# andrewhou1/GeomConsistentFR

Hardware: AMD Instinct MI355X
Metric: ray_steps_per_sec (higher is better)
Workload: dtype f64+f32

## Files before the change

### geomconsistentfr_amd/csrc/gcfr_march.hpp

```cpp
#pragma once

#include "gcfr_device.hpp"
#include "gcfr_mutants.hpp"

#include "../../include/gcfr.h"

#include <atomic>
#include <cstddef>
#include <type_traits>

namespace gcfr {

struct ShadowArgs {
    const float *depth;
    const uint8_t *mask;
    const float *light_pt;
    const double *t_table;
    float *min_dist;
    int32_t *argmin;
    int32_t mask_batch, L, H, W, N;
    int32_t tiles_x, tiles_per_image;
    float bonus, bx_lo, bx_hi, by_lo, by_hi;
};

struct RayConst {
    float x, y, zb;
    float dx, dy;
    float BCx, BCy, BCz;
    double x64, y64, dx64, dy64, halfW, halfH;
    int H, W;
};

__device__ inline float ray_sample(const RayConst &rc, double t, __amdgpu_buffer_rsrc_t zr,
                                   __amdgpu_buffer_rsrc_t mr, bool &masked)
{
    const int W = rc.W, H = rc.H;
    const double sx = rc.x64 + t * rc.dx64;
    const double sy = rc.y64 + t * rc.dy64;
    const int col_r = (int)(__builtin_rint(sx) + rc.halfW);
    const int row_r = (int)(rc.halfH - __builtin_rint(sy));
    const double ux = (sx + rc.halfW) - 0.0001;
    const double uy = (rc.halfH - sy) - 0.0001;
    const double fxd = __builtin_floor(ux), gxd = __builtin_ceil(ux);
    const double fyd = __builtin_floor(uy), gyd = __builtin_ceil(uy);
    int fx = (int)fxd, gx = (int)gxd, fy = (int)fyd, gy = (int)gyd;
    const double wx0 = gxd - ux, wx1 = ux - fxd;
    const double wy0 = gyd - uy, wy1 = uy - fyd;
    fx += (fx >> 31) & W;
    fy += (fy >> 31) & H;
    const int rowf = fy * W, rowg = gy * W;
    const double zUL = buf_load_f32(zr, (rowf + fx) << 2);
    const double zUR = buf_load_f32(zr, (rowf + gx) << 2);
    const double zLL = buf_load_f32(zr, (rowg + fx) << 2);
    const double zLR = buf_load_f32(zr, (rowg + gx) << 2);
    const uint32_t mk = buf_load_u8(mr, row_r * W + col_r);
    const double up = zUL * wx0 + zUR * wx1;
    const double low = zLL * wx0 + zLR * wx1;
    const double zA = up * wy0 + low * wy1;
    const float Ax = (float)(ux - rc.halfW), Ay = (float)(rc.halfH - uy), Az = (float)zA;
    const float BAx = Ax - rc.x, BAy = Ay - rc.y, BAz = Az - rc.zb;
    const float Xx = __builtin_fmaf(BAy, rc.BCz, -(BAz * rc.BCy));
    const float Xy = __builtin_fmaf(BAz, rc.BCx, -(BAx * rc.BCz));
    const float Xz = __builtin_fmaf(BAx, rc.BCy, -(BAy * rc.BCx));
    masked = (mk == 0);
    return ((Xx * Xx + Xy * Xy) + Xz * Xz) + kEps4;
}

__device__ inline int first_tied_sample(const RayConst &rc, const double *t_table, __amdgpu_buffer_rsrc_t zr,
                                        __amdgpu_buffer_rsrc_t mr, bool tie, int prevk, float den, float d)
{
    int first = prevk;
    int k_hi = tie ? prevk : 0;
    for (int off = 32; off > 0; off >>= 1)
        k_hi = max(k_hi, __shfl_xor(k_hi, off));
    k_hi = __builtin_amdgcn_readfirstlane(k_hi);
    bool found = !tie;
    for (int k = 0; k < k_hi; ++k) {
        bool masked;
        const float S = ray_sample(rc, t_table[k], zr, mr, masked);
        const bool hit = !found && (k < prevk) && !masked && (__builtin_sqrtf(S) / den == d);
        first = hit ? k : first;
        found = found || hit;
    }
    return first;
}



struct PrepassLights {
    const float *light_raw = nullptr;
    float *unit_out = nullptr, *light_pt_out = nullptr;
    int L = 0, clamp_z = 0;
    float clamp_min = 0.0f, light_distance = 0.0f;
};

constexpr int kBBoxInit = 0x7f7f7f7f;

template <int CTRL, int ROW_MASK>
__device__ inline int dpp_min_step(int v)
{
    const int moved = __builtin_amdgcn_update_dpp(0x7fffffff, v, CTRL, ROW_MASK, 0xf, false);
    return min(v, moved);
}
__device__ inline int wave_min_i32(int v)
{
    v = dpp_min_step<0x111, 0xf>(v);
    v = dpp_min_step<0x112, 0xf>(v);
    v = dpp_min_step<0x114, 0xf>(v);
    v = dpp_min_step<0x118, 0xf>(v);
    v = dpp_min_step<0x142, 0xa>(v);
    v = dpp_min_step<0x143, 0xc>(v);
    return __builtin_amdgcn_readlane(v, 63);
}

__device__ inline int f32_sortable(float f)
{
    const int i = __builtin_bit_cast(int, f);
    return i ^ ((i >> 31) & 0x7fffffff);
}
__device__ inline float f32_unsortable(int i)
{
    return __builtin_bit_cast(float, i ^ ((i >> 31) & 0x7fffffff));
}

template <class TablePtrT>
__device__ inline int zb_log2_stride(int H, int W, int N, TablePtrT t_table, int group, bool *fits = nullptr)
{
    if (fits)
        *fits = false;
    if (N < 2)
        return 3;
    const float step = fabsf((float)((t_table[N - 1] - t_table[0]) / (double)(N - 1)));
    const float fd = (float)(group - 1) * step * (float)max(H, W) * 1.002f;
    const int need = (int)fminf(fmaxf(fd, 0.0f), 1024.0f) + GCFR_M(22, 1, 3);
    int ls = 3;
    while ((1 << ls) < need && ls < 5)
        ++ls;
    if (fits)
        *fits = (1 << ls) >= need;
    return ls;
}

__host__ __device__ inline int zb_max_tiles(int H, int W) { return ((H >> 3) + 1) * ((W >> 3) + 1) + 1; }
__host__ __device__ inline int zb_stride(int H, int W) { return (zb_max_tiles(H, W) + 63) & ~63; }
constexpr int kHorizonDim = 1024;
constexpr int kHorizonBands = 4;
__host__ __device__ inline bool hz_shape_ok(int H, int W) { return ((W & 3) == 0) && W <= kHorizonDim && H <= kHorizonDim; }
__host__ __device__ inline int zb_slot(int H, int W) { return hz_shape_ok(H, W) ? zb_stride(H, W) + 4 * kHorizonDim : zb_stride(H, W); }

__device__ inline float row_sum_f32(float v)
{
    v += __builtin_bit_cast(float, __builtin_amdgcn_update_dpp(0, __builtin_bit_cast(int, v), 0x111, 0xf, 0xf, false));
    v += __builtin_bit_cast(float, __builtin_amdgcn_update_dpp(0, __builtin_bit_cast(int, v), 0x112, 0xf, 0xf, false));
    v += __builtin_bit_cast(float, __builtin_amdgcn_update_dpp(0, __builtin_bit_cast(int, v), 0x114, 0xf, 0xf, false));
    v += __builtin_bit_cast(float, __builtin_amdgcn_update_dpp(0, __builtin_bit_cast(int, v), 0x118, 0xf, 0xf, false));
    return v;
}
__device__ inline float lane_value(float v, int lane)
{
    return __builtin_bit_cast(float, __builtin_amdgcn_readlane(__builtin_bit_cast(int, v), lane));
}


constexpr int kQueueSlot = 64;
enum { kTfOk = 0, kTfStride = 1, kTfTabs = 2, kTfTfirst = 3, kTfInvDt = 4 };
constexpr int kStatChunk = 16384;
__host__ __device__ inline int stat_chunk_shift(int H, int W)
{
    const int raw = (H * W + kStatChunk - 1) >> 14;
    return (raw > 8 && raw <= 16) ? 15 : 14;
}
__host__ __device__ inline int stat_chunk_px(int H, int W) { return 1 << stat_chunk_shift(H, W); }
__host__ __device__ inline int n_stat_chunks(int H, int W)
{
    const int sh = stat_chunk_shift(H, W);
    return (H * W + (1 << sh) - 1) >> sh;
}
static_assert(kStatChunk == 1 << 14, "stat_chunk_shift() spells kStatChunk as a shift");


struct MarchEpilogueArgs {
    float *min_dist;
    int32_t *argmin;
    float bonus, bx_lo, bx_hi, by_lo, by_hi;
    const float *normals;
    const float *albedo;
    const float *ambient;
    float *shadow_w, *full, *final_shading, *rendered;
    float intensity;
    NormalsArgs nrm;
    float *normals_out;
};

struct ShadowQuadArgs {
    const float *depth;
    const float4 *quad;
    const int *bbox;
    const int *diag;
    const float4 *zb;
    const int *zrange;
    const int *mones;
    int *tflag;
    const uint8_t *mask;
    const uint32_t *reserved0;
    const float *light_pt;
    const double *t_table;
    unsigned long long *counters;
    int32_t mask_batch, B, L, H, W, N;
    int32_t tiles_x, tiles_y;
    int32_t bl_offset;
    int32_t hz_off;
    MarchEpilogueArgs epi;
};

typedef const __attribute__((address_space(4))) ShadowQuadArgs *ArgPtr;
typedef const __attribute__((address_space(4))) MarchEpilogueArgs *EpiPtr;
__device__ __forceinline__ ArgPtr kernel_args()
{
    return (ArgPtr)__builtin_amdgcn_kernarg_segment_ptr();
}
template <class T>
__device__ __forceinline__ T launder(T p)
{
    asm volatile("" : "+s"(p));
    return p;
}

constexpr double kRintMagic = 6755399441055744.0;
typedef float f32x4 __attribute__((ext_vector_type(4)));

__device__ inline int lo32(double v)
{
    return (int)(unsigned)(__builtin_bit_cast(unsigned long long, v) & 0xffffffffull);
}

enum { kCntTiles, kCntGroupsNominal, kCntGroupsVisited, kCntBoundTests, kCntBodies, kCntLaneSamples, kCntEarlyExit,
       kCntTieRemarch, kCntSamplesInRange, kCntBoundsGivenUp, kCntVisitsAfterLastBody, kCntVisitsBeforeFirstBody,
       kCntTrailEnter, kCntTrailSkips, kCntTrailLeave, kCntRoughSamples, kCntWaveSamples, kCntWaveSamplesTaken, kCntLaneTakes,
       kCntAuditBoundChecks, kCntAuditBoundViol, kCntAuditTermChecks, kCntAuditTermViol, kCntAuditMaskedChecks, kCntAuditMaskedViol,
       kCntAuditSafeViol, kCntAuditMaxUse, kCntUsed };
static_assert(kCntUsed <= GCFR_N_COUNTERS, "gcfr_options.counters holds GCFR_N_COUNTERS tallies");
#if defined(GCFR_AUDIT) && !defined(GCFR_COUNTERS)
#error "-DGCFR_AUDIT needs -DGCFR_COUNTERS"
#endif
#ifdef GCFR_COUNTERS
#define GCFR_COUNT(i, n) (cnt[i] += (unsigned)(n))
#else
#define GCFR_COUNT(i, n) ((void)0)
#endif

struct ImageStats {
    int r_min, c_min, r_max, c_max;
    int s_min, s_max, d_min, d_max;
    int gz_lo_s, gz_nhi_s;
    int mask_all_ones;
};
__device__ inline ImageStats reduce_image_stats(ArgPtr a, int b, int lane, bool want_z)
{
    const int n = n_stat_chunks(a->H, a->W);
    if (n <= 8) {
        typedef const __attribute__((address_space(4))) int *ConstI32Ptr;
        const ConstI32Ptr sb = (ConstI32Ptr)(unsigned long long)a->bbox + 4 * (size_t)(a->mask_batch == 1 ? 0 : b) * n;
        const ConstI32Ptr sz = (ConstI32Ptr)(unsigned long long)a->zrange + 2 * (size_t)b * n;
        const ConstI32Ptr so = (ConstI32Ptr)(unsigned long long)a->mones + (size_t)(a->mask_batch == 1 ? 0 : b) * n;
        const ConstI32Ptr sd = (ConstI32Ptr)(unsigned long long)a->diag + 4 * (size_t)(a->mask_batch == 1 ? 0 : b) * n;
        int d0 = kBBoxInit, d1 = kBBoxInit, d2 = kBBoxInit, d3 = kBBoxInit;
        int m0 = kBBoxInit, m1 = kBBoxInit, m2 = kBBoxInit, m3 = kBBoxInit, z0 = 0x7fffffff, z1 = 0x7fffffff, ones = 1;
#pragma unroll
        for (int j = 0; j < 8; ++j) {
            if (j < n) {
                m0 = min(m0, sb[4 * j + 0]);
                m1 = min(m1, sb[4 * j + 1]);
                m2 = min(m2, sb[4 * j + 2]);
                m3 = min(m3, sb[4 * j + 3]);
                ones = min(ones, so[j]);
                d0 = min(d0, sd[4 * j + 0]);
                d1 = min(d1, sd[4 * j + 1]);
                d2 = min(d2, sd[4 * j + 2]);
                d3 = min(d3, sd[4 * j + 3]);
                if (want_z) {
                    z0 = min(z0, sz[2 * j + 0]);
                    z1 = min(z1, sz[2 * j + 1]);
                }
            }
        }
        ImageStats st;
        st.r_min = m0;
        st.c_min = m1;
        st.r_max = -m2;
        st.c_max = -m3;
        st.gz_lo_s = z0;
        st.gz_nhi_s = z1;
        st.mask_all_ones = ones;
        st.s_min = d0;
        st.s_max = -d1;
        st.d_min = d2;
        st.d_max = -d3;
        return st;
    }
    const int4 *pb = (const int4 *)a->bbox + (size_t)(a->mask_batch == 1 ? 0 : b) * n;
    const int2 *pz = (const int2 *)a->zrange + (size_t)b * n;
    const int *po = a->mones + (size_t)(a->mask_batch == 1 ? 0 : b) * n;
    const int4 *pd = (const int4 *)a->diag + (size_t)(a->mask_batch == 1 ? 0 : b) * n;
    int4 m = make_int4(kBBoxInit, kBBoxInit, kBBoxInit, kBBoxInit), dg = m;
    int2 mz = make_int2(0x7fffffff, 0x7fffffff);
    int ones = 1;
    for (int j = lane; j < n; j += 64) {
        ones = min(ones, po[j]);
        const int4 v = pb[j];
        m.x = min(m.x, v.x);
        m.y = min(m.y, v.y);
        m.z = min(m.z, v.z);
        m.w = min(m.w, v.w);
        const int4 w = pd[j];
        dg.x = min(dg.x, w.x);
        dg.y = min(dg.y, w.y);
        dg.z = min(dg.z, w.z);
        dg.w = min(dg.w, w.w);
        if (want_z) {
            const int2 vz = pz[j];
            mz.x = min(mz.x, vz.x);
            mz.y = min(mz.y, vz.y);
        }
    }
    ImageStats st;
    st.r_min = wave_min_i32(m.x);
    st.c_min = wave_min_i32(m.y);
    st.r_max = -wave_min_i32(m.z);
    st.c_max = -wave_min_i32(m.w);
    st.gz_lo_s = want_z ? wave_min_i32(mz.x) : 0x7fffffff;
    st.gz_nhi_s = want_z ? wave_min_i32(mz.y) : 0x7fffffff;
    st.mask_all_ones = wave_min_i32(ones);
    st.s_min = wave_min_i32(dg.x);
    st.s_max = -wave_min_i32(dg.y);
    st.d_min = wave_min_i32(dg.z);
    st.d_max = -wave_min_i32(dg.w);
    return st;
}

__device__ inline int fresh_lane_id()
{
    int l;
    asm volatile("v_mbcnt_lo_u32_b32 %0, -1, 0\n\tv_mbcnt_hi_u32_b32 %0, -1, %0" : "=v"(l));
    return l;
}

enum { kModeInline = 0, kModeFull = 1, kModeRough = 2 };
#ifndef GCFR_ROUGH_CHUNK
#define GCFR_ROUGH_CHUNK 3
#endif
#ifndef GCFR_ROUGH_CHUNK_ARGMIN
#define GCFR_ROUGH_CHUNK_ARGMIN 3
#endif
template <int TILE_W, bool EVEN_HALF, bool WANT_ARGMIN, int DEPTH, bool FUSE_SHADE, int SPLIT, bool ALL_ONES = false, bool OWN = false,
          int MODE = kModeInline>
__device__ __forceinline__ bool march_tile(ArgPtr a, const int bl, const int qy, const int tx,
                                           const ImageStats &st)
{
    static_assert(MODE == kModeInline || SPLIT == 0, "full / rough pairs: the grid schedule's kernels");
    constexpr int TILE_H = 64 / TILE_W;
    static_assert(SPLIT == 0 || SPLIT == 1, "SPLIT: 0 = one wave per tile, 1 = the workgroup's four waves split the sample range");
    static_assert(!(OWN && (SPLIT != 0 || ALL_ONES)), "pixels = mask: the grid schedule only");
    const int H = a->H, W = a->W, L = a->L;
    typedef const __attribute__((address_space(4))) double *TablePtr;
    typedef const __attribute__((address_space(4))) float *ConstF32Ptr;
    typedef const __attribute__((address_space(4))) int *ConstI32Ptr;
    const TablePtr tt = (TablePtr)(unsigned long long)a->t_table;
    const int lane = fresh_lane_id();
    const int wave = __builtin_amdgcn_readfirstlane((int)(threadIdx.x >> 6));
    constexpr bool KSPLIT = SPLIT == 1;
    constexpr bool TRAIL = !KSPLIT;
    constexpr bool ROUGH = MODE == kModeRough;
    const int chunk = KSPLIT ? (a->N + 3) >> 2 : a->N;
    const int k_lo = KSPLIT ? wave * chunk : 0;
    const int N = KSPLIT ? min(a->N, k_lo + chunk) : a->N;
#ifdef GCFR_COUNTERS
    unsigned cnt[kCntUsed] = {};
    unsigned cnt_since_body = 0, cnt_had_body = 0;
    const unsigned long long trace_t0 = __builtin_amdgcn_s_memrealtime(), trace_c0 = __builtin_amdgcn_s_memtime();
#endif

    const int b = bl / L;
    const int l = bl - b * L;
    int r = qy * TILE_H + lane / TILE_W;
    int c = tx * TILE_W + (lane % TILE_W);
    const bool valid = (r < H) && (c < W);
    r = valid ? r : H - 1;
    c = valid ? c : W - 1;

    const size_t P = (size_t)H * W;
    const int Wp = W + 1;
    const size_t Pq = (size_t)(H + 1) * Wp;
    const __amdgpu_buffer_rsrc_t qr = make_rsrc(a->quad + (size_t)b * Pq, (int)(Pq * 16));
    const __amdgpu_buffer_rsrc_t mr =
        make_rsrc(a->mask + (size_t)(a->mask_batch == 1 ? 0 : b) * P, (int)P);

    const bool own_off = GCFR_M(17, false &&, ) OWN && (!valid || (buf_load_u8(mr, __mul24(r, W) + c) == 0));

    const ConstF32Ptr lp = (ConstF32Ptr)(unsigned long long)a->light_pt;
    const float Cx = lp[3 * bl + 0], Cy = lp[3 * bl + 1], Cz = lp[3 * bl + 2];
    const Box box = image_box(H, W);
    const LightCase lc = classify_light(Cx, Cy, box);
    const float halfWf = W / 2.0f, halfHf = H / 2.0f;
    const double halfW = W / 2.0, halfH = H / 2.0;
    const int halfWi = W / 2, halfHi = H / 2;

    const float x = (float)c - halfWf, y = halfHf - (float)r;
    const float zb = a->depth[(size_t)b * P + (size_t)r * W + c];
    float Ex, Ey;
    end_point(x, y, Cx, Cy, box, lc, Ex, Ey);
    const float dxf = Ex - x, dyf = Ey - y;
    const float BCx = Cx - x, BCy = Cy - y, BCz = Cz - zb;
    const bool finite_ray = (dxf - dxf == 0.0f) && (dyf - dyf == 0.0f);
    const double x64 = x, y64 = y;
    const double dx64 = finite_ray ? (double)dxf : 0.0, dy64 = finite_ray ? (double)dyf : 0.0;
    const double Mx = EVEN_HALF ? kRintMagic + halfW : kRintMagic;
    const double My = EVEN_HALF ? kRintMagic + halfH : kRintMagic;
    const int quad_origin = (Wp + 1) << 4;
#ifdef GCFR_AUDIT
    RayConst arc;
    arc.H = H;
    arc.W = W;
    arc.halfW = halfW;
    arc.halfH = halfH;
    arc.x = x;
    arc.y = y;
    arc.zb = zb;
    arc.dx = dxf;
    arc.dy = dyf;
    arc.BCx = BCx;
    arc.BCy = BCy;
    arc.BCz = BCz;
    arc.x64 = x64;
    arc.y64 = y64;
    arc.dx64 = dx64;
    arc.dy64 = dy64;
    const __amdgpu_buffer_rsrc_t azr = make_rsrc(a->depth + (size_t)b * P, (int)(P * 4));
    bool audit_dead = false;
    auto audit_S = [&](int k, bool &masked) -> float {
        const float S = ray_sample(arc, (double)tt[k], azr, mr, masked);
        masked = masked || audit_dead;
        return S;
    };
    auto audit_count = [&](int slot, bool pred) { cnt[slot] += (unsigned)__builtin_popcountll(__builtin_amdgcn_ballot_w64(pred)); };
    auto audit_masked = [&](int k_from, int k_to, bool claim) {
        for (int k = k_from; k < k_to; ++k) {
            bool m;
            (void)audit_S(k, m);
            audit_count(kCntAuditMaskedChecks, claim && finite_ray);
            audit_count(kCntAuditMaskedViol, claim && finite_ray && !m);
        }
    };
#endif
    const ConstI32Ptr tfl = (ConstI32Ptr)(unsigned long long)a->tflag;
    const bool t_increasing = (a->N >= 2) && (tfl[kTfOk] != 0);
    bool use_zb = !ROUGH && (a->zb != nullptr) && t_increasing;
    if (MODE == kModeFull && !use_zb)
        return true;
    const int zrec = tfl[kTfStride];
    const int zls = use_zb ? (zrec & 0xff) : 3;
    const int zntw = (W >> zls) + 1;
    const float nrm = __builtin_amdgcn_sqrtf(BCx * BCx + BCy * BCy);
    const float c1 = BCz * ((dxf * BCx + dyf * BCy) * __builtin_amdgcn_rcpf(nrm));
    const float t_abs = __builtin_bit_cast(float, tfl[kTfTabs]);
#ifndef GCFR_GIVEUP_FACTOR
#define GCFR_GIVEUP_FACTOR 0.5f
#endif
    if (use_zb) {
        const int own = __mul24((qy * TILE_H) >> zls, zntw) + ((tx * TILE_W) >> zls);
        const ConstF32Ptr rec = (ConstF32Ptr)(unsigned long long)a->zb + 4 * ((size_t)b * zb_slot(H, W) + own);
        const float band = rec[3] - rec[2];
        const bool hopeless = !(fabsf(c1) * t_abs >= GCFR_GIVEUP_FACTOR * nrm * band);
        if (__builtin_amdgcn_ballot_w64(!hopeless) == 0ull) {
            if (MODE == kModeFull)
                return true;
            use_zb = false;
            GCFR_COUNT(kCntBoundsGivenUp, 1);
        }
    }

    float bestS = __builtin_inff();
    int besti = -1;
    float prevS = __builtin_inff();
    int prevk = -1;
    bool any_masked = false;

    int k_begin = k_lo, k_end = N;
    const int gz_lo_s = st.gz_lo_s, gz_nhi_s = st.gz_nhi_s;
    int lane_last = (OWN && own_off) ? -1 : a->N - 1;
    if (t_increasing) {
        const int r_min = st.r_min, c_min = st.c_min, r_max = st.r_max, c_max = st.c_max;
        int lane_lo = a->N, lane_hi = -1;
        if (r_min != kBBoxInit && !(OWN && own_off)) {
            const float X0 = __builtin_fmaf(0.5f, (float)(2 * c_min - W), -GCFR_M(1, 0.49f, 0.51f)), X1 = __builtin_fmaf(0.5f, (float)(2 * c_max - W), GCFR_M(1, 0.49f, 0.51f));
            const float Y0 = __builtin_fmaf(0.5f, (float)(H - 2 * r_max), -GCFR_M(1, 0.49f, 0.51f)), Y1 = __builtin_fmaf(0.5f, (float)(H - 2 * r_min), GCFR_M(1, 0.49f, 0.51f));
            float ta = -3.0e38f, tb = 3.0e38f;
            bool empty = !finite_ray;
            auto slab = [&](float p, float dp, float lo, float hi) {
                const bool still = dp == 0.0f;
                const float inv = __builtin_amdgcn_rcpf(dp);
                const float t1 = (lo - p) * inv, t2 = (hi - p) * inv;
                const float whole = ((p < lo) || (p > hi)) ? 3.0e38f : -3.0e38f;
                ta = fmaxf(ta, still ? whole : fminf(t1, t2));
                tb = fminf(tb, still ? -whole : fmaxf(t1, t2));
            };
            slab(x, dxf, X0, X1);
            slab(y, dyf, Y0, Y1);
            if (st.mask_all_ones == 0) {
                const int ws = W + H, wd = W - H;
                const float U0 = __builtin_fmaf(0.5f, (float)(2 * st.s_min - ws), -GCFR_M(2, 0.98f, 1.02f)), U1 = __builtin_fmaf(0.5f, (float)(2 * st.s_max - ws), GCFR_M(2, 0.98f, 1.02f));
                const float V0 = __builtin_fmaf(0.5f, (float)(2 * st.d_min - wd), -GCFR_M(2, 0.98f, 1.02f)), V1 = __builtin_fmaf(0.5f, (float)(2 * st.d_max - wd), GCFR_M(2, 0.98f, 1.02f));
                slab(x - y, dxf - dyf, U0, U1);
                slab(x + y, dxf + dyf, V0, V1);
            }
            if (!empty && ta <= tb) {
                const float t_first = __builtin_bit_cast(float, tfl[kTfTfirst]);
                const float inv_dt = __builtin_bit_cast(float, tfl[kTfInvDt]);
                const float ka = (ta - t_first) * inv_dt, kb = (tb - t_first) * inv_dt;
                lane_lo = (int)fminf(fmaxf(floorf(ka) - 1.0f, 0.0f), (float)a->N);
                lane_hi = (int)fmaxf(fminf(ceilf(kb) + 1.0f, (float)(a->N - 1)), -1.0f);
            }
        }
        lane_last = lane_hi;
#ifdef GCFR_AUDIT
        audit_dead = OWN && own_off;
        for (int k = 0; k < a->N; ++k) {
            bool m;
            (void)audit_S(k, m);
            const bool claim = finite_ray && ((k < lane_lo) || (k > lane_hi));
            audit_count(kCntAuditMaskedChecks, claim);
            audit_count(kCntAuditMaskedViol, claim && !m);
        }
#endif
        const int w_lo = __builtin_amdgcn_readfirstlane(wave_min_i32(lane_lo));
        const int w_hi = -__builtin_amdgcn_readfirstlane(wave_min_i32(-lane_hi));
        const int nb = max(k_begin, w_lo), ne = min(k_end, w_hi + 1);
        any_masked = GCFR_M(24, false, (nb > k_begin) || (ne < k_end));
        k_begin = nb;
        k_end = ne;
    }
    if (k_begin >= k_end)
        use_zb = false;
    GCFR_COUNT(kCntTiles, 1);
    if (ROUGH)
        GCFR_COUNT(kCntBoundsGivenUp, 1);
    GCFR_COUNT(kCntGroupsNominal, (N - k_lo + DEPTH - 1) / DEPTH);
    GCFR_COUNT(kCntSamplesInRange, k_end > k_begin ? k_end - k_begin : 0);

    const bool zfits = use_zb && ((zrec & 0x100) != 0);
    const bool zb_trusted = __builtin_amdgcn_readfirstlane((int)zfits) != 0;
    const __amdgpu_buffer_rsrc_t zr =
        make_rsrc(a->zb + (size_t)b * zb_slot(H, W), zb_slot(H, W) * (int)sizeof(float4));
    auto dir_f32 = [&](float &dxl, float &dyl) {
        if (WANT_ARGMIN) {
            dxl = finite_ray ? dxf : 0.0f;
            dyl = finite_ray ? dyf : 0.0f;
            return;
        }
        double dx_l = dx64, dy_l = dy64;
        asm volatile("" : "+v"(dx_l), "+v"(dy_l));
        dxl = (float)dx_l;
        dyl = (float)dy_l;
    };
    float Kerr = __builtin_inff();
    float gz_cap = __builtin_inff();
    float safeS = 0.0f;
    if (use_zb) {
        const float gz_lo = f32_unsortable(gz_lo_s), gz_hi = -f32_unsortable(gz_nhi_s);
        const float rr = fmaxf(fmaxf(fabsf(gz_lo - zb), fabsf(gz_hi - zb)), fmaxf(fabsf(zb), (float)max(H, W)));
        const float K1 = GCFR_M(3, 0.0f, 4e-3f * fabsf(BCz) + 1e-6f * fabsf(c1) * t_abs);
        const float K2 = GCFR_M(4, 0.0f, 1e-6f * nrm + 2e-7f * ((fabsf(BCx) + fabsf(BCy)) + fabsf(BCz)));
        const float K = __builtin_fmaf(K2, rr, K1) + GCFR_M(5, 0.0f, nrm * (1.2e-2f + 8e-6f * (float)max(H, W)));
        if ((nrm > 0.0f) && finite_ray && (K - K == 0.0f)) {
            Kerr = GCFR_M(23, 0.0f, K);
        }
        if (a->hz_off >= 0) {
            const ConstF32Ptr e = (ConstF32Ptr)(unsigned long long)a->zb + 4 * ((size_t)b * zb_slot(H, W) + zb_stride(H, W) + kHorizonDim);
            gz_cap = fmaxf(fmaxf(e[0], e[1]), fmaxf(e[2], e[3]));
        } else {
            gz_cap = GCFR_M(25, gz_hi, fmaxf(gz_hi, 0.0f));
        }
        gz_cap = __builtin_bit_cast(float, __builtin_amdgcn_readfirstlane(__builtin_bit_cast(int, gz_cap)));
        const float den2 = (BCx * BCx + BCy * BCy) + BCz * BCz;
        const float s_lane = (den2 - den2 == 0.0f) ? GCFR_M(9, 1.02e12f, 0.98e12f) * den2 : 0.0f;
        safeS = f32_unsortable(__builtin_amdgcn_readfirstlane(wave_min_i32(f32_sortable(s_lane))));
    }

    const int zb_sentinel = (zb_max_tiles(H, W) - 1) << 4;
    auto zb_fetch = [&](int ca, int ra, int cb, int rb) -> f32x4 {
        const int cmin = min(ca, cb), cmax = max(ca, cb), rmin = min(ra, rb), rmax = max(ra, rb);
        const int tj = cmin >> zls, ti = rmin >> zls;
        int off = (__mul24(ti, zntw) + tj) << 4;
        if (!zb_trusted) {
            const bool covered = (cmin >= 0) && (rmin >= 0) && (cmax <= W - 1) && (rmax <= H - 1) &&
                                 (cmax + 2 <= ((tj + 2) << zls) - 1) && (rmax + 2 <= ((ti + 2) << zls) - 1);
            off = covered ? off : zb_sentinel;
        }
        return __builtin_bit_cast(f32x4, __builtin_amdgcn_raw_buffer_load_b128(zr, off, 0, 0));
    };

    auto mask_offset = [&](double sx, double sy, int &col_r, int &row_r) -> int {
        if (EVEN_HALF) {
            col_r = lo32(sx + Mx);
            row_r = lo32(My - sy);
        } else {
            col_r = lo32(sx + Mx) + halfWi;
            row_r = halfHi - lo32(sy + My);
        }
        return __mul24(row_r, W) + col_r;
    };

    auto clampk = [&](int k) { return k < k_end ? k : k_end - 1; };
#ifdef GCFR_AUDIT
    auto audit_safe = [&](bool claim) {
        const float den_a = sqrt_rn_normal(((BCx * BCx + BCy * BCy) + BCz * BCz) + kEps4);
        const float d_a = sqrt_rn_normal(bestS) / den_a;
        audit_count(kCntAuditSafeViol, claim && finite_ray && !(d_a < kMaskedDistance));
    };
    auto audit_finish = [&](int k_from, bool by_bound, float gd, float slack, bool by_last) {
        for (int k = k_from; k < k_end; ++k) {
            bool m;
            const float S = audit_S(k, m);
            audit_count(kCntAuditTermChecks, by_bound && !m);
            audit_count(kCntAuditTermViol, by_bound && !m && (S < gd * gd * slack));
            audit_count(kCntAuditMaskedChecks, !by_bound && by_last && finite_ray);
            audit_count(kCntAuditMaskedViol, !by_bound && by_last && finite_ray && !m);
        }
        audit_safe(by_bound);
    };
#endif
    struct Prefetched {
        uint32_t m[DEPTH];
        f32x4 z;
    };
    double tq[DEPTH];
    double tc0 = 0.0, tc3 = 0.0;
    auto load_tq = [&](int kfirst) {
#pragma unroll
        for (int j = 0; j < DEPTH; ++j)
            tq[j] = tt[clampk(kfirst + j)];
    };
    auto pos_tq = [&](int j, double &sx, double &sy) {
        sx = x64 + tq[j] * dx64;
        sy = y64 + tq[j] * dy64;
    };
    auto prefetch = [&](Prefetched &p) {
        int cj[DEPTH], rj[DEPTH];
        if (ALL_ONES) {
#pragma unroll
            for (int j = 0; j < DEPTH; ++j)
                p.m[j] = 1u;
            if (use_zb) {
                double px, py;
                pos_tq(0, px, py);
                (void)mask_offset(px, py, cj[0], rj[0]);
                pos_tq(DEPTH - 1, px, py);
                (void)mask_offset(px, py, cj[DEPTH - 1], rj[DEPTH - 1]);
                p.z = zb_fetch(cj[0], rj[0], cj[DEPTH - 1], rj[DEPTH - 1]);
            }
            return;
        }
#pragma unroll
        for (int j = 0; j < DEPTH; ++j) {
            double px, py;
            pos_tq(j, px, py);
            p.m[j] = buf_load_u8(mr, mask_offset(px, py, cj[j], rj[j]));
        }
        if (use_zb)
            p.z = zb_fetch(cj[0], rj[0], cj[DEPTH - 1], rj[DEPTH - 1]);
    };
    auto finish_check = [&](int k0, double tn64, bool check_finished) -> bool {
        if (check_finished && use_zb && k0 + DEPTH < k_end) {
            const float tn = (float)tn64;
            float nrm_l = nrm;
            asm volatile("" : "+v"(nrm_l));
            const float gd = __builtin_fmaf(c1, tn, -(__builtin_fmaf(nrm_l, gz_cap, -(nrm_l * zb)) + Kerr));
            const float bS = bestS;
            const bool finished = (GCFR_M(11, true, (c1 > 0.0f)) && (gd > 0.0f) && (gd * gd * GCFR_M(7, GCFR_MUT_SLACK_VALUE, 0.998f) > bS) && (bS < safeS)) ||
                                  (lane_last < k0 + DEPTH GCFR_M(26, + 1, ));
            if (__builtin_amdgcn_ballot_w64(!finished) == 0ull) {
                any_masked |= (lane_last < k0 + DEPTH GCFR_M(26, + 1, ));
                GCFR_COUNT(kCntEarlyExit, 1);
#ifdef GCFR_AUDIT
                audit_finish(k0 + DEPTH, GCFR_M(11, true, (c1 > 0.0f)) && (gd > 0.0f) && (gd * gd * GCFR_M(7, GCFR_MUT_SLACK_VALUE, 0.998f) > bS) && (bS < safeS),
                             gd, GCFR_M(7, GCFR_MUT_SLACK_VALUE, 0.998f), lane_last < k0 + DEPTH GCFR_M(26, + 1, ));
#endif
                return false;
            }
        }
        return true;
    };
    auto bound_cw = [&](const f32x4 &cz, double ta64, double tb64, int k0) -> bool {
            GCFR_COUNT(kCntBoundTests, 1);
            const float ta = (float)ta64, tb = (float)tb64;
            float zb_l = zb;
            if (TRAIL && !WANT_ARGMIN)
                asm volatile("" : "+v"(zb_l));
            const float Qz = nrm * zb_l;
            const float Ta = c1 * ta, Tb = c1 * tb;
            const float Tlo = fminf(Ta, Tb), Thi = fmaxf(Ta, Tb);
            float dxl, dyl;
            dir_f32(dxl, dyl);
            const float A0 = __builtin_fmaf(cz.x, x, cz.y * y), A1 = __builtin_fmaf(cz.x, dxl, cz.y * dyl);
            const float E = __builtin_fmaf(nrm, A1, -c1);
            const float Flo = __builtin_fmaf(nrm, A0 + cz.z, -Qz), Fhi = __builtin_fmaf(nrm, A0 + cz.w, -Qz);
            const float eA = ta * E, eB = GCFR_M(29, ta, tb) * E;
            const float gap = fmaxf(Flo + fminf(eA, eB), -(Fhi + fmaxf(eA, eB)));
            const float gap0 = fmaxf(-Qz - Thi, Tlo + Qz);
            const float g = GCFR_M(10, gap, fminf(gap, gap0)) - Kerr;
#ifdef GCFR_AUDIT
            for (int j = 0; j < DEPTH; ++j) {
                bool m;
                const float S = audit_S(clampk(k0 + j), m);
                const bool claim = (g > 0.0f) && !m;
                audit_count(kCntAuditBoundChecks, claim);
                audit_count(kCntAuditBoundViol, claim && (S < g * g * GCFR_M(6, 1.002f, 0.998f)));
                const float use = claim ? ((g + Kerr) - __builtin_sqrtf(S)) / Kerr : 0.0f;
                const int use_m = (int)fminf(fmaxf(use * 1000.0f, 0.0f), 1.0e6f);
                cnt[kCntAuditMaxUse] = max(cnt[kCntAuditMaxUse], (unsigned)(-wave_min_i32(-use_m)));
            }
#else
            (void)k0;
#endif
            return (g > 0.0f) && (g * g * GCFR_M(6, 1.002f, 0.998f) > bestS);
    };
    auto eval_sample = [&](int k, bool masked, double uxj, double uyj, double fxj, double fyj, const f32x4 &q) {
        const double gxd = __builtin_ceil(uxj), gyd = __builtin_ceil(uyj);
        const double wx0 = gxd - uxj, wx1 = uxj - fxj;
        const double wy0 = gyd - uyj, wy1 = uyj - fyj;
        const double zUL = q.x, zUR = q.y, zLL = q.z, zLR = q.w;
        const double up = zUL * wx0 + zUR * wx1;
        const double low = zLL * wx0 + zLR * wx1;
        const double zA = up * wy0 + low * wy1;
        const float Ax = (float)(uxj - halfW), Ay = (float)(halfH - uyj), Az = (float)zA;
        const float BAx = Ax - x, BAy = Ay - y, BAz = Az - zb;
        const float Xx = __builtin_fmaf(BAy, BCz, -(BAz * BCy));
        const float Xy = __builtin_fmaf(BAz, BCx, -(BAx * BCz));
        const float Xz = __builtin_fmaf(BAx, BCy, -(BAy * BCx));
        const float S = ((Xx * Xx + Xy * Xy) + Xz * Xz) + kEps4;
        const bool take = !masked && (S < bestS);
#ifdef GCFR_COUNTERS
        {
            const unsigned long long tk = __builtin_amdgcn_ballot_w64(take);
            cnt[kCntWaveSamples] += 1u;
            cnt[kCntWaveSamplesTaken] += (tk != 0ull) ? 1u : 0u;
            cnt[kCntLaneTakes] += (unsigned)__builtin_popcountll(tk);
        }
#endif
        if (WANT_ARGMIN) {
            prevS = take ? bestS : prevS;
            prevk = take ? besti : prevk;
            besti = take ? k : besti;
        }
        bestS = take ? S : bestS;
    };
    bool all_lazy = false;
    auto consume = [&](int k0, const uint32_t (&cm)[DEPTH], const f32x4 &cz, double ta64, double tb64, double tn64,
                       bool check_finished, auto lazy, bool cw_in) -> bool {
        constexpr bool LAZY = decltype(lazy)::value;
        if (TRAIL)
            all_lazy = false;
        if (!LAZY)
            GCFR_COUNT(kCntGroupsVisited, 1);
#ifdef GCFR_COUNTERS
        ++cnt_since_body;
#endif
        const bool dead = OWN && (lane_last < 0);
        bool none = true;
#pragma unroll
        for (int j = 0; j < DEPTH; ++j) {
            none = none && (cm[j] == 0);
            any_masked |= (cm[j] == 0);
        }
        none = none || dead;
        bool run_body = __builtin_amdgcn_ballot_w64(!none) != 0ull;
        if (LAZY) {
            run_body = __builtin_amdgcn_ballot_w64(!none && !cw_in) != 0ull;
        } else if (run_body && use_zb) {
            const bool cannot_win = bound_cw(cz, ta64, tb64, k0);
            run_body = __builtin_amdgcn_ballot_w64(!none && !cannot_win) != 0ull;
            if (TRAIL)
                all_lazy = !run_body && __builtin_amdgcn_ballot_w64(!((cannot_win && GCFR_M(18, true, (bestS < safeS))) || (lane_last < k0))) == 0ull;
        }
#ifndef GCFR_INFER_BODY_CHUNK
#define GCFR_INFER_BODY_CHUNK 1
#endif
        constexpr int GCFR_BODY_CHUNK = KSPLIT ? DEPTH : (WANT_ARGMIN && DEPTH >= 2 ? 2 : GCFR_INFER_BODY_CHUNK);
        if (run_body) {
          GCFR_COUNT(kCntBodies, 1);
#ifdef GCFR_COUNTERS
          if (!cnt_had_body)
              cnt[kCntVisitsBeforeFirstBody] += cnt_since_body - 1;
          cnt_had_body = 1;
          cnt_since_body = 0;
#endif
#ifdef GCFR_COUNTERS
#pragma unroll
          for (int j = 0; j < DEPTH; ++j)
              cnt[kCntLaneSamples] += (unsigned)__builtin_popcountll(__builtin_amdgcn_ballot_w64(cm[j] != 0));
#endif
#pragma unroll
          for (int h0 = 0; h0 < DEPTH; h0 += GCFR_BODY_CHUNK) {
            double ux[DEPTH], uy[DEPTH], fxd[DEPTH], fyd[DEPTH];
            f32x4 qv[DEPTH];
#pragma unroll
            for (int j = h0; j < h0 + GCFR_BODY_CHUNK && j < DEPTH; ++j) {
                constexpr bool CARRIED = FUSE_SHADE || WANT_ARGMIN;
                const double tj = (CARRIED && j == 0) ? ta64 : ((CARRIED && j == DEPTH - 1) ? tb64 : (double)tt[clampk(k0 + j)]);
                const double sx = x64 + tj * dx64, sy = y64 + tj * dy64;
                ux[j] = (sx + halfW) - 0.0001;
                uy[j] = (halfH - sy) - 0.0001;
                fxd[j] = __builtin_floor(ux[j]);
                fyd[j] = __builtin_floor(uy[j]);
                const int fx = (int)fxd[j], fy = (int)fyd[j];
                const int texel = __mul24(fy, Wp) + fx;
                qv[j] = __builtin_bit_cast(
                    f32x4, __builtin_amdgcn_raw_buffer_load_b128(qr, (texel << 4) + quad_origin, 0, 0));
            }
#pragma unroll
            for (int j = h0; j < h0 + GCFR_BODY_CHUNK && j < DEPTH; ++j)
                eval_sample(clampk(k0 + j), (cm[j] == 0) || dead, ux[j], uy[j], fxd[j], fyd[j], qv[j]);
          }
        }
        return finish_check(k0, tn64, check_finished);
    };
    auto group = [&](int k0, const Prefetched &cur, Prefetched &nxt, bool check_finished) -> bool {
        const double ta64 = tc0, tb64 = tc3;
        tc0 = tq[0];
        tc3 = tq[DEPTH - 1];
        prefetch(nxt);
        load_tq(k0 + 2 * DEPTH);
        return consume(k0, cur.m, cur.z, ta64, tb64, tc0, check_finished, std::false_type{}, false);
    };

    if (ROUGH) {
        constexpr int CH = WANT_ARGMIN ? GCFR_ROUGH_CHUNK_ARGMIN : GCFR_ROUGH_CHUNK;
        double tr[CH];
        auto load_tr = [&](int kfirst) {
#pragma unroll
            for (int j = 0; j < CH; ++j)
                tr[j] = tt[clampk(kfirst + j)];
        };
        if (k_begin < k_end)
            load_tr(k_begin);
        for (int k0 = k_begin; k0 < k_end; k0 += CH) {
            GCFR_COUNT(kCntRoughSamples, min(CH, k_end - k0));
            double ux[CH], uy[CH], fxd[CH], fyd[CH];
            f32x4 qv[CH];
            uint32_t mk[CH];
#pragma unroll
            for (int j = 0; j < CH; ++j) {
                const double tj = tr[j];
                const double sx = x64 + tj * dx64, sy = y64 + tj * dy64;
                int cr, rr;
                const int moff = mask_offset(sx, sy, cr, rr);
                mk[j] = ALL_ONES ? 1u : buf_load_u8(mr, moff);
                ux[j] = (sx + halfW) - 0.0001;
                uy[j] = (halfH - sy) - 0.0001;
                fxd[j] = __builtin_floor(ux[j]);
                fyd[j] = __builtin_floor(uy[j]);
                const int texel = __mul24((int)fyd[j], Wp) + (int)fxd[j];
                qv[j] = __builtin_bit_cast(f32x4, __builtin_amdgcn_raw_buffer_load_b128(qr, (texel << 4) + quad_origin, 0, 0));
            }
            load_tr(k0 + CH);
#pragma unroll
            for (int j = 0; j < CH; ++j) {
                const bool masked = (mk[j] == 0) || (OWN && (lane_last < 0));
                any_masked |= masked;
                eval_sample(clampk(k0 + j), masked, ux[j], uy[j], fxd[j], fyd[j], qv[j]);
            }
        }
    } else {
    Prefetched bufA, bufB;
    bufA.z = bufB.z = f32x4{0.0f, 0.0f, -__builtin_inff(), __builtin_inff()};
    const int k_first = k_begin;
    if (k_first < k_end) {
        load_tq(k_first);
        tc0 = tq[0];
        tc3 = tq[DEPTH - 1];
        prefetch(bufA);
        load_tq(k_first + DEPTH);
    }
    int k_trail = k_end;
    f32x4 zcur = bufA.z;
    for (int k0 = k_first; k0 < k_end; k0 += 2 * DEPTH) {
        if (!group(k0, bufA, bufB, false))
            break;
        if (k0 + DEPTH >= k_end)
            break;
        if (TRAIL && all_lazy) {
            k_trail = k0 + DEPTH;
            zcur = bufB.z;
            break;
        }
        if (!group(k0 + DEPTH, bufB, bufA, true))
            break;
        if (TRAIL && all_lazy && k0 + 2 * DEPTH < k_end) {
            k_trail = k0 + 2 * DEPTH;
            zcur = bufA.z;
            break;
        }
    }
    if (TRAIL) {
        if (k_trail < k_end)
            GCFR_COUNT(kCntTrailEnter, 1);
        auto record_of = [&](double t_first, double t_last) -> f32x4 {
            int ca, ra, cb, rb;
            (void)mask_offset(x64 + t_first * dx64, y64 + t_first * dy64, ca, ra);
            (void)mask_offset(x64 + t_last * dx64, y64 + t_last * dy64, cb, rb);
            return zb_fetch(ca, ra, cb, rb);
        };
        for (int k0 = k_trail; k0 < k_end; k0 += DEPTH) {
            const double ta64 = tc0, tb64 = tc3;
            tc0 = tq[0];
            tc3 = tq[DEPTH - 1];
            const f32x4 znext = record_of(tc0, tc3);
            load_tq(k0 + 2 * DEPTH);
            const bool check = (((k0 - k_trail) / DEPTH) & 1) != 0;
            const int hz_off = check && (k0 + DEPTH < k_end) ? launder(a)->hz_off : -1;
            const bool check_hz = hz_off >= 0;
            const float tn = (float)tc0;
            const bool cw = bound_cw(zcur, ta64, tb64, k0);
            const bool gone = lane_last < k0 GCFR_M(27, + 1, );
            GCFR_COUNT(kCntGroupsVisited, 1);
            if (__builtin_amdgcn_ballot_w64(!((cw && GCFR_M(18, true, (bestS < safeS))) || gone)) == 0ull) {
                any_masked |= gone;
                GCFR_COUNT(kCntTrailSkips, 1);
#ifdef GCFR_AUDIT
                audit_safe(cw && !gone);
                audit_masked(k0, min(k0 + DEPTH, k_end), gone);
#endif
#ifdef GCFR_COUNTERS
                ++cnt_since_body;
#endif
                if (check_hz) {
                    float dxl, dyl;
                    dir_f32(dxl, dyl);
                    const int ci = (int)__builtin_floorf(__builtin_fmaf(tn, dxl, x)), ri = (int)__builtin_floorf(-__builtin_fmaf(tn, dyl, y));
                    constexpr int C = kHorizonDim / 2, M = kHorizonDim - 1;
                    const int ic = (dxl >= 0.0f) ? kHorizonDim + min(max(ci + C, 0), M) : min(max(ci + C, 0), M);
                    const int ir = (dyl > 0.0f) ? 2 * kHorizonDim + min(max(ri + C, 0), M) : 3 * kHorizonDim + min(max(ri + C, 0), M);
                    const f32x4 zc4 = __builtin_bit_cast(f32x4, __builtin_amdgcn_raw_buffer_load_b128(zr, hz_off + (ic << 4), 0, 0));
                    const f32x4 zr4 = __builtin_bit_cast(f32x4, __builtin_amdgcn_raw_buffer_load_b128(zr, hz_off + (ir << 4), 0, 0));
                    const float zc = fmaxf(fmaxf(zc4.x, zc4.y), fmaxf(zc4.z, zc4.w)), zr_ = fmaxf(fmaxf(zr4.x, zr4.y), fmaxf(zr4.z, zr4.w));
                    float nrm_l = nrm;
                    asm volatile("" : "+v"(nrm_l));
                    const float Dc = __builtin_fmaf(nrm_l, fminf(zc, zr_), -(nrm_l * zb)) + Kerr;
                    const float gd = __builtin_fmaf(c1, tn, -Dc);
                    const bool past = lane_last < k0 + DEPTH GCFR_M(26, + 1, );
                    const bool finished = (GCFR_M(11, true, (c1 > 0.0f)) && (gd > 0.0f) && (gd * gd * GCFR_M(8, GCFR_MUT_SLACK_VALUE, 0.998f) > bestS) && (bestS < safeS)) || past;
                    if (__builtin_amdgcn_ballot_w64(!finished) == 0ull) {
                        any_masked |= past;
                        GCFR_COUNT(kCntEarlyExit, 1);
#ifdef GCFR_AUDIT
                        audit_finish(k0 + DEPTH, GCFR_M(11, true, (c1 > 0.0f)) && (gd > 0.0f) && (gd * gd * GCFR_M(8, GCFR_MUT_SLACK_VALUE, 0.998f) > bestS) && (bestS < safeS),
                                     gd, GCFR_M(8, GCFR_MUT_SLACK_VALUE, 0.998f), past);
#endif
                        break;
                    }
                } else if (!finish_check(k0, tc0, check)) {
                    break;
                }
            } else {
                GCFR_COUNT(kCntTrailLeave, 1);
                uint32_t cm[DEPTH];
#pragma unroll
                for (int j = 0; j < DEPTH; ++j) {
                    const double tj = (j == 0) ? ta64 : ((j == DEPTH - 1) ? tb64 : (double)tt[clampk(k0 + j)]);
                    int cj, rj;
                    cm[j] = ALL_ONES ? 1u : buf_load_u8(mr, mask_offset(x64 + tj * dx64, y64 + tj * dy64, cj, rj));
                }
                if (!consume(k0, cm, zcur, ta64, tb64, tc0, check, std::true_type{}, cw))
                    break;
                zcur = record_of(tc0, tc3);
                continue;
            }
            zcur = znext;
        }
    }
    }

    if (KSPLIT) {
        __shared__ float sS[4][64], sPS[4][64];
        __shared__ int sK[4][64], sPK[4][64];
        __shared__ uint8_t sM[4][64];
        sS[wave][lane] = bestS;
        sK[wave][lane] = besti;
        sPS[wave][lane] = prevS;
        sPK[wave][lane] = prevk;
        sM[wave][lane] = any_masked ? 1 : 0;
        __syncthreads();
        if (wave != 0)
            return false;
#pragma unroll
        for (int q = 1; q < 4; ++q) {
            const float Sq = sS[q][lane];
            const bool take = Sq < bestS;
            const float PSq = sPS[q][lane];
            const bool local_pred = PSq < bestS;
            prevS = take ? (local_pred ? PSq : bestS) : prevS;
            prevk = take ? (local_pred ? sPK[q][lane] : besti) : prevk;
            bestS = take ? Sq : bestS;
            besti = take ? sK[q][lane] : besti;
            any_masked |= (sM[q][lane] != 0);
        }
    }

    float BCx_e = BCx;
    asm volatile("" : "+v"(BCx_e));
    const int lane_e = fresh_lane_id();
    const int r_e = qy * TILE_H + lane_e / TILE_W, c_e = tx * TILE_W + (lane_e % TILE_W);
    const bool valid_e = (r_e < H) && (c_e < W);
    r = valid_e ? r_e : H - 1;
    c = valid_e ? c_e : W - 1;
    const size_t pix = (size_t)r * W + c;
    const size_t o = (size_t)bl * P + pix;
    const EpiPtr ep = launder((EpiPtr)&a->epi);
    float *const min_dist = ep->min_dist;
    int32_t *const argmin = WANT_ARGMIN ? ep->argmin : nullptr;
    const float bonus = ep->bonus, bx_lo = ep->bx_lo, bx_hi = ep->bx_hi, by_lo = ep->by_lo, by_hi = ep->by_hi;
    const float *const normals = FUSE_SHADE ? ep->normals : nullptr;
    const float *const albedo = FUSE_SHADE ? ep->albedo : nullptr;
    float *const shadow_w = FUSE_SHADE ? ep->shadow_w : nullptr, *const full = FUSE_SHADE ? ep->full : nullptr;
    float *const final_shading = FUSE_SHADE ? ep->final_shading : nullptr, *const rendered = FUSE_SHADE ? ep->rendered : nullptr;
    float *const normals_out = FUSE_SHADE ? ep->normals_out : nullptr;
    const float intensity = FUSE_SHADE ? ep->intensity : 0.0f;
    const float amb = FUSE_SHADE ? ((ConstF32Ptr)(unsigned long long)ep->ambient)[bl] : 0.0f;
    NormalsArgs na = {};
    float zs[9], n[3], alb[3];
    if (FUSE_SHADE) {
        na.H = H;
        na.W = W;
        na.inv_fx = ep->nrm.inv_fx;
        na.inv_fy = ep->nrm.inv_fy;
        na.cx = ep->nrm.cx;
        na.cy = ep->nrm.cy;
        na.z_offset = ep->nrm.z_offset;
        na.negate_y = ep->nrm.negate_y;
        if (normals) {
            const float *nrm_in = normals + (size_t)b * 3 * P + pix;
            n[0] = nrm_in[0];
            n[1] = nrm_in[P];
            n[2] = nrm_in[2 * P];
        } else {
            load_depth_stencil(H, W, a->depth + (size_t)b * P, r, c, zs);
        }
        const float *alb_in = albedo + (size_t)b * 3 * P + pix;
#pragma unroll
        for (int ch = 0; ch < 3; ++ch)
            alb[ch] = alb_in[ch * P];
    }

    const float den = sqrt_rn_normal(((BCx_e * BCx_e + BCy * BCy) + BCz * BCz) + kEps4);
    float d = sqrt_rn_normal(bestS) / den;
    if (WANT_ARGMIN) {
        const bool tie = GCFR_M(16, false &&, ) (prevk >= 0) && (sqrt_rn_normal(prevS) / den == d);
        if (__builtin_amdgcn_ballot_w64(tie) != 0ull) {
            GCFR_COUNT(kCntTieRemarch, 1);
            RayConst rc;
            rc.H = H;
            rc.W = W;
            rc.halfW = halfW;
            rc.halfH = halfH;
            rc.x = x;
            rc.y = y;
            rc.zb = zb;
            dir_f32(rc.dx, rc.dy);
            rc.BCx = BCx;
            rc.BCy = BCy;
            rc.BCz = BCz;
            rc.x64 = x64;
            rc.y64 = y64;
            rc.dx64 = dx64;
            rc.dy64 = dy64;
            const int first = first_tied_sample(rc, a->t_table, make_rsrc(a->depth + (size_t)b * P, (int)(P * 4)), mr,
                                                tie, prevk, den, d);
            besti = tie ? first : besti;
        }
    }
    if (any_masked && !(d < kMaskedDistance)) {
        d = kMaskedDistance;
        besti = -1;
    }
    if (OWN && (lane_last < 0)) {
        d = kMaskedDistance;
        besti = -1;
    }
    if (!finite_ray)
        d = __builtin_nanf("");
    const bool inside = (Cx >= bx_lo) && (Cx <= bx_hi) && (Cy >= by_lo) && (Cy <= by_hi);
    if (inside)
        d = d + bonus;
    if (!valid_e)
        return false;
    auto store = [](auto *p, auto v) {
        if (!WANT_ARGMIN)
            __builtin_nontemporal_store(v, p);
        else
            *p = v;
    };
    store(min_dist + o, d);
    if (WANT_ARGMIN)
        store(argmin + o, besti);
    if (FUSE_SHADE) {
        if (!normals) {
            unit_normal_from(na, zs, r, c, n);
            if (normals_out && l == 0) {
                float *no = normals_out + (size_t)b * 3 * P + pix;
                store(no, n[0]);
                store(no + P, n[1]);
                store(no + 2 * P, n[2]);
            }
        }
        const Shaded sh = shade_pixel(x, y, zb, n[0], n[1], n[2], Cx, Cy, Cz, amb, intensity, d);
        if (shadow_w)
            store(shadow_w + o, sh.w);
        if (full)
            store(full + o, sh.full);
        if (final_shading)
            store(final_shading + o, sh.fin);
        float *ren = rendered + (size_t)bl * 3 * P + pix;
#pragma unroll
        for (int ch = 0; ch < 3; ++ch)
            store(ren + ch * P, alb[ch] * sh.fin);
    }
#ifdef GCFR_COUNTERS
    if (a->counters && lane == 0 && !(KSPLIT && wave != 0)) {
        cnt[kCntVisitsAfterLastBody] += cnt_since_body;
#ifndef GCFR_TRACE_ONLY
#pragma unroll
        for (int i = 0; i < kCntUsed; ++i) {
            if (i == kCntAuditMaxUse)
                atomicMax(a->counters + i, (unsigned long long)cnt[i]);
            else
                atomicAdd(a->counters + i, (unsigned long long)cnt[i]);
        }
#endif
        unsigned long long *rec = a->counters + GCFR_N_COUNTERS + 4 * ((size_t)(bl * a->tiles_y + qy) * a->tiles_x + tx);
        const unsigned hw_id = __builtin_amdgcn_s_getreg((31 << 11) | 4);
        const unsigned xcc_id = __builtin_amdgcn_s_getreg((31 << 11) | 20);
        rec[0] = trace_t0;
        rec[1] = __builtin_amdgcn_s_memrealtime();
        rec[2] = __builtin_amdgcn_s_memtime() - trace_c0;
        rec[3] = (unsigned long long)hw_id | ((unsigned long long)(xcc_id & 0xf) << 32) |
                 ((unsigned long long)(cnt[kCntBodies] & 0xfff) << 36) | ((unsigned long long)(cnt[kCntGroupsVisited] & 0xfff) << 48);
    }
#endif
    return false;
}

#ifndef GCFR_MARCH_WAVES_PER_EU
#define GCFR_MARCH_WAVES_PER_EU 6
#endif
#ifndef GCFR_MARCH_ARGMIN_WAVES_PER_EU
#define GCFR_MARCH_ARGMIN_WAVES_PER_EU 5
#endif

template <int TILE_W, bool EVEN_HALF, bool WANT_ARGMIN, int DEPTH, bool FUSE_SHADE, bool OWN = false>
__device__ __forceinline__ void march_grid(ArgPtr a)
{
    const int wave = __builtin_amdgcn_readfirstlane((int)(threadIdx.x >> 6));
    const int tx = (int)blockIdx.x * 4 + wave;
    const int bl = a->bl_offset + (int)blockIdx.z;
    const bool want_z = (a->zb != nullptr);
    const ImageStats st = reduce_image_stats(a, bl / a->L, threadIdx.x & 63, want_z);
    if (tx >= a->tiles_x)
        return;
    bool rough;
    if (st.mask_all_ones != 0)
        rough = march_tile<TILE_W, EVEN_HALF, WANT_ARGMIN, DEPTH, FUSE_SHADE, 0, true, false, kModeFull>(a, bl, (int)blockIdx.y, tx, st);
    else
        rough = march_tile<TILE_W, EVEN_HALF, WANT_ARGMIN, DEPTH, FUSE_SHADE, 0, false, OWN, kModeFull>(a, bl, (int)blockIdx.y, tx, st);
    if (GCFR_M(15, false &&, ) __builtin_amdgcn_readfirstlane((int)rough) != 0) {
        const ArgPtr a2 = WANT_ARGMIN ? a : launder(a);
        const int bl2 = WANT_ARGMIN ? bl : a2->bl_offset + (int)blockIdx.z;
        const ImageStats st2 = WANT_ARGMIN ? st : reduce_image_stats(a2, bl2 / a2->L, threadIdx.x & 63, false);
        if (st2.mask_all_ones != 0)
            march_tile<TILE_W, EVEN_HALF, WANT_ARGMIN, DEPTH, FUSE_SHADE, 0, true, false, kModeRough>(a2, bl2, (int)blockIdx.y, tx, st2);
        else
            march_tile<TILE_W, EVEN_HALF, WANT_ARGMIN, DEPTH, FUSE_SHADE, 0, false, OWN, kModeRough>(a2, bl2, (int)blockIdx.y, tx, st2);
    }
}

enum { kSchedGrid = 0 };

template <int SCHED, int TILE_W, bool EVEN_HALF, bool WANT_ARGMIN, int DEPTH, bool FUSE_SHADE, bool OWN = false>
__device__ __forceinline__ void march_dispatch()
{
    static_assert(SCHED == kSchedGrid, "the product library has the grid schedule only");
    march_grid<TILE_W, EVEN_HALF, WANT_ARGMIN, DEPTH, FUSE_SHADE, OWN>(kernel_args());
}

template <int TILE_W, bool EVEN_HALF, int DEPTH, bool FUSE_SHADE, int SCHED>
__global__ __launch_bounds__(256)
__attribute__((amdgpu_waves_per_eu(GCFR_MARCH_WAVES_PER_EU, GCFR_MARCH_WAVES_PER_EU))) void shadow_fwd_quad_kernel(ShadowQuadArgs)
{
    march_dispatch<SCHED, TILE_W, EVEN_HALF, false, DEPTH, FUSE_SHADE>();
}
template <int TILE_W, bool EVEN_HALF, int DEPTH, bool FUSE_SHADE, int SCHED>
__global__ __launch_bounds__(256)
__attribute__((amdgpu_waves_per_eu(GCFR_MARCH_ARGMIN_WAVES_PER_EU, GCFR_MARCH_ARGMIN_WAVES_PER_EU))) void shadow_fwd_quad_argmin_kernel(ShadowQuadArgs)
{
    march_dispatch<SCHED, TILE_W, EVEN_HALF, true, DEPTH, FUSE_SHADE>();
}
template <int TILE_W, bool EVEN_HALF, int DEPTH, bool FUSE_SHADE, int SCHED>
__global__ __launch_bounds__(256)
__attribute__((amdgpu_waves_per_eu(GCFR_MARCH_ARGMIN_WAVES_PER_EU, GCFR_MARCH_ARGMIN_WAVES_PER_EU))) void shadow_fwd_quad_argmin_own_kernel(ShadowQuadArgs)
{
    march_dispatch<SCHED, TILE_W, EVEN_HALF, true, DEPTH, FUSE_SHADE, true>();
}
template <int TILE_W, bool EVEN_HALF, bool WANT_ARGMIN, int DEPTH, bool FUSE_SHADE>
__global__ __launch_bounds__(256) void shadow_fwd_quad_ksplit_kernel(ShadowQuadArgs)
{
    const ArgPtr a = kernel_args();
    const int bl = a->bl_offset + (int)blockIdx.z;
    const ImageStats st = reduce_image_stats(a, bl / a->L, threadIdx.x & 63, a->zb != nullptr);
    march_tile<TILE_W, EVEN_HALF, WANT_ARGMIN, DEPTH, FUSE_SHADE, 1>(a, bl, (int)blockIdx.y, (int)blockIdx.x, st);
}


enum Schedule { kGrid = kSchedGrid, kKSplit, kGridOwn };

template <int TILE_W, int DEPTH, bool FUSE>
static void launch_quad4(const ShadowQuadArgs &a, bool even_half, bool want_argmin, Schedule sch, dim3 grid, hipStream_t st)
{
#define GCFR_LAUNCH(KERNEL, ...) hipLaunchKernelGGL((KERNEL<TILE_W, __VA_ARGS__>), grid, dim3(256), 0, st, a)
    if (sch == kKSplit) {
        if (even_half) {
            if (want_argmin)
                GCFR_LAUNCH(shadow_fwd_quad_ksplit_kernel, true, true, DEPTH, FUSE);
            else
                GCFR_LAUNCH(shadow_fwd_quad_ksplit_kernel, true, false, DEPTH, FUSE);
        } else {
            if (want_argmin)
                GCFR_LAUNCH(shadow_fwd_quad_ksplit_kernel, false, true, DEPTH, FUSE);
            else
                GCFR_LAUNCH(shadow_fwd_quad_ksplit_kernel, false, false, DEPTH, FUSE);
        }
    } else if (sch == kGridOwn) {
        if (even_half)
            GCFR_LAUNCH(shadow_fwd_quad_argmin_own_kernel, true, DEPTH, FUSE, kSchedGrid);
        else
            GCFR_LAUNCH(shadow_fwd_quad_argmin_own_kernel, false, DEPTH, FUSE, kSchedGrid);
    } else {
        if (even_half) {
            if (want_argmin)
                GCFR_LAUNCH(shadow_fwd_quad_argmin_kernel, true, DEPTH, FUSE, kSchedGrid);
            else
                GCFR_LAUNCH(shadow_fwd_quad_kernel, true, DEPTH, FUSE, kSchedGrid);
        } else {
            if (want_argmin)
                GCFR_LAUNCH(shadow_fwd_quad_argmin_kernel, false, DEPTH, FUSE, kSchedGrid);
            else
                GCFR_LAUNCH(shadow_fwd_quad_kernel, false, DEPTH, FUSE, kSchedGrid);
        }
    }
#undef GCFR_LAUNCH
}

template <int TILE_W, int DEPTH>
static void launch_quad3(const ShadowQuadArgs &a, bool even_half, bool want_argmin, Schedule sch, dim3 grid, hipStream_t st)
{
    if (a.epi.rendered)
        launch_quad4<TILE_W, DEPTH, true>(a, even_half, want_argmin, sch, grid, st);
    else
        launch_quad4<TILE_W, DEPTH, false>(a, even_half, want_argmin, sch, grid, st);
}

typedef void (*MarchUnitFn)(const ShadowQuadArgs &a, bool even_half, bool want_argmin, Schedule sch, dim3 grid, hipStream_t st);
#define GCFR_MARCH_UNIT_NAME_(TW, G) launch_march_##TW##_##G
#define GCFR_MARCH_UNIT_NAME(TW, G) GCFR_MARCH_UNIT_NAME_(TW, G)
#define GCFR_DECLARE_MARCH_UNIT(TW, G)                                                                              \
    void GCFR_MARCH_UNIT_NAME(TW, G)(const ShadowQuadArgs &a, bool even_half, bool want_argmin, Schedule sch, dim3 grid, \
                                     hipStream_t st);
GCFR_DECLARE_MARCH_UNIT(16, 4)
#ifndef GCFR_FAST_BUILD
GCFR_DECLARE_MARCH_UNIT(16, 2)
GCFR_DECLARE_MARCH_UNIT(16, 1)
GCFR_DECLARE_MARCH_UNIT(8, 4)
GCFR_DECLARE_MARCH_UNIT(8, 2)
GCFR_DECLARE_MARCH_UNIT(8, 1)
GCFR_DECLARE_MARCH_UNIT(32, 4)
GCFR_DECLARE_MARCH_UNIT(32, 2)
GCFR_DECLARE_MARCH_UNIT(32, 1)
GCFR_DECLARE_MARCH_UNIT(64, 4)
GCFR_DECLARE_MARCH_UNIT(64, 2)
GCFR_DECLARE_MARCH_UNIT(64, 1)
#endif

}
```

Before: 2444 billion.

## Software-pipeline shadow body loads and defer next-group prefetch into body

For the non-argmin, fused-shade, non-split inline path, the per-group body now issues its texel buffer loads two samples ahead of evaluation, so loads overlap the arithmetic of earlier samples. The prefetch of the next group's mask/depth records and t-table values moves from before the body to a point late in the body (or straight after the skip when no body runs). The aim is to hide memory latency and reduce register pressure from prefetching early. It adds register-pinning asm barriers and recomputes floors, which may cost extra VGPRs or instructions, and changes the timing of the prefetches.

```diff
diff --git a/geomconsistentfr_amd/csrc/gcfr_march.hpp b/geomconsistentfr_amd/csrc/gcfr_march.hpp
--- a/geomconsistentfr_amd/csrc/gcfr_march.hpp
+++ b/geomconsistentfr_amd/csrc/gcfr_march.hpp
@@ -349,6 +349,9 @@
 #ifndef GCFR_ROUGH_CHUNK
 #define GCFR_ROUGH_CHUNK 3
 #endif
+#ifndef GCFR_BODY_PIPELINE
+#define GCFR_BODY_PIPELINE 1
+#endif
 #ifndef GCFR_ROUGH_CHUNK_ARGMIN
 #define GCFR_ROUGH_CHUNK_ARGMIN 3
 #endif
@@ -371,6 +374,7 @@
     constexpr bool KSPLIT = SPLIT == 1;
     constexpr bool TRAIL = !KSPLIT;
     constexpr bool ROUGH = MODE == kModeRough;
+    constexpr bool PIPE = GCFR_BODY_PIPELINE && !WANT_ARGMIN && !KSPLIT && !ROUGH && FUSE_SHADE && DEPTH >= 2;
     const int chunk = KSPLIT ? (a->N + 3) >> 2 : a->N;
     const int k_lo = KSPLIT ? wave * chunk : 0;
     const int N = KSPLIT ? min(a->N, k_lo + chunk) : a->N;
@@ -756,7 +760,7 @@
     };
     bool all_lazy = false;
     auto consume = [&](int k0, const uint32_t (&cm)[DEPTH], const f32x4 &cz, double ta64, double tb64, double tn64,
-                       bool check_finished, auto lazy, bool cw_in) -> bool {
+                       bool check_finished, auto lazy, bool cw_in, auto late) -> bool {
         constexpr bool LAZY = decltype(lazy)::value;
         if (TRAIL)
             all_lazy = false;
@@ -799,6 +803,7 @@
           for (int j = 0; j < DEPTH; ++j)
               cnt[kCntLaneSamples] += (unsigned)__builtin_popcountll(__builtin_amdgcn_ballot_w64(cm[j] != 0));
 #endif
+          if (!(PIPE && !LAZY)) {
 #pragma unroll
           for (int h0 = 0; h0 < DEPTH; h0 += GCFR_BODY_CHUNK) {
             double ux[DEPTH], uy[DEPTH], fxd[DEPTH], fyd[DEPTH];
@@ -821,6 +826,41 @@
             for (int j = h0; j < h0 + GCFR_BODY_CHUNK && j < DEPTH; ++j)
                 eval_sample(clampk(k0 + j), (cm[j] == 0) || dead, ux[j], uy[j], fxd[j], fyd[j], qv[j]);
           }
+          } else {
+            uint32_t mflags = 0u;
+#pragma unroll
+            for (int j = 0; j < DEPTH; ++j)
+                mflags |= (cm[j] == 0 ? 1u : 0u) << j;
+            mflags = dead ? ~0u : mflags;
+            asm volatile("" : "+v"(mflags));
+            double ux[DEPTH], uy[DEPTH];
+            f32x4 qv[DEPTH];
+            auto issue = [&](int j) {
+                constexpr bool CARRIED = FUSE_SHADE || WANT_ARGMIN;
+                const double tj = (CARRIED && j == 0) ? ta64 : ((CARRIED && j == DEPTH - 1) ? tb64 : (double)tt[clampk(k0 + j)]);
+                const double sx = x64 + tj * dx64, sy = y64 + tj * dy64;
+                ux[j] = (sx + halfW) - 0.0001;
+                uy[j] = (halfH - sy) - 0.0001;
+                const int fx = (int)__builtin_floor(ux[j]), fy = (int)__builtin_floor(uy[j]);
+                const int texel = __mul24(fy, Wp) + fx;
+                qv[j] = __builtin_bit_cast(
+                    f32x4, __builtin_amdgcn_raw_buffer_load_b128(qr, (texel << 4) + quad_origin, 0, 0));
+                asm volatile("" : "+v"(ux[j]), "+v"(uy[j]));
+            };
+            issue(0);
+            if (DEPTH > 1)
+                issue(1);
+#pragma unroll
+            for (int j = 0; j < DEPTH; ++j) {
+                eval_sample(clampk(k0 + j), ((mflags >> j) & 1u) != 0u, ux[j], uy[j], __builtin_floor(ux[j]), __builtin_floor(uy[j]), qv[j]);
+                if (j + 2 < DEPTH)
+                    issue(j + 2);
+                if (j == (DEPTH >= 3 ? DEPTH - 3 : 0))
+                    late();
+            }
+          }
+        } else if (PIPE) {
+            late();
         }
         return finish_check(k0, tn64, check_finished);
     };
@@ -828,9 +868,15 @@
         const double ta64 = tc0, tb64 = tc3;
         tc0 = tq[0];
         tc3 = tq[DEPTH - 1];
-        prefetch(nxt);
-        load_tq(k0 + 2 * DEPTH);
-        return consume(k0, cur.m, cur.z, ta64, tb64, tc0, check_finished, std::false_type{}, false);
+        if (!PIPE) {
+            prefetch(nxt);
+            load_tq(k0 + 2 * DEPTH);
+            return consume(k0, cur.m, cur.z, ta64, tb64, tc0, check_finished, std::false_type{}, false, []() {});
+        }
+        return consume(k0, cur.m, cur.z, ta64, tb64, tc0, check_finished, std::false_type{}, false, [&]() {
+            prefetch(nxt);
+            load_tq(k0 + 2 * DEPTH);
+        });
     };
 
     if (ROUGH) {
@@ -970,7 +1016,7 @@
                     int cj, rj;
                     cm[j] = ALL_ONES ? 1u : buf_load_u8(mr, mask_offset(x64 + tj * dx64, y64 + tj * dy64, cj, rj));
                 }
-                if (!consume(k0, cm, zcur, ta64, tb64, tc0, check, std::true_type{}, cw))
+                if (!consume(k0, cm, zcur, ta64, tb64, tc0, check, std::true_type{}, cw, []() {}))
                     break;
                 zcur = record_of(tc0, tc3);
                 continue;
```

Measured after the change: 2512 billion, median of 6. +2.8%, better.
